# Griffan/VerifyBamID

Measured on AMD Instinct MI355X. Metric: llk_evals_per_sec, higher is better.
Workload: dtype f64; 1 GPU; synthetic pileup 100000 markers x depth 30, --NumPC 4 (BASELINE.json configs[2] shape); parallelism=1 GPU, rccl_world_size=1, launched_by=single process, reads=2999230, active_markers=100000, distinct_codes=42, device=gfx950:sramecc+:xnack-

## Files before the change

### verifybamid_amd/csrc/eval_body.h

```cpp
#ifndef VB2_EVAL_BODY_H_
#define VB2_EVAL_BODY_H_

#include "llk_kernels.h"

#include <hip/hip_runtime.h>

#include "kernel_debug.h"

#include <type_traits>
namespace vb2 {

__device__ __forceinline__ void pair_of(int p, int& g1, int& g2)
{
    g1 = p >> 1;
    const int lo = p & 1;
    g2 = lo + (lo >= g1 ? 1 : 0);
}

__device__ __forceinline__ double wave_sum(double v)
{
    {
        const unsigned hi = (unsigned)__double2hiint(v), lo = (unsigned)__double2loint(v);
        const auto h = __builtin_amdgcn_permlane32_swap(hi, hi, false, false);
        const auto l = __builtin_amdgcn_permlane32_swap(lo, lo, false, false);
// ... 209 lines not shown
__device__ __forceinline__ double prob_entry(double alpha, double p_err, int g1, int g2)
{
    const double p_ok = 1.0 - p_err;
    const double e1 = (double)g1 * (1.0 / 6.0), e2 = (double)g2 * (1.0 / 6.0);
    const double n1 = 1.0 - 0.5 * (double)g1, n2 = 1.0 - 0.5 * (double)g2;
    const double one_minus_alpha = 1.0 - alpha;
    double val = (alpha * e1 + one_minus_alpha * e2) * p_err +
                 (alpha * n1 + one_minus_alpha * n2) * p_ok;
    return val >= 0.0 ? val : __builtin_nan("");
}

__device__ __forceinline__ void initial_gf(double af, double* gf)
{
    af = vmin_f64(vmax_f64(af, 0.00005), 0.99995);
    gf[0] = (1 - af) * (1 - af);
    gf[1] = 2 * (af) * (1 - af);
    gf[2] = af * af;
}


constexpr int kExpTabDoubles = 64 * 32;
constexpr int kPrefetch = 8;
constexpr int kPrefetchL2 = 2;

__device__ __forceinline__ void lane_map(int lane, int& m, int& g)
{
    const int q = (lane >> 2) & 7;
    const int nib = (0x76452310u >> (4 * q)) & 7;
    g = (nib & 1) + 2 * (lane >> 5);
    m = ((nib >> 1) << 2) + (lane & 3);
}
__device__ __forceinline__ int lane_of(int m, int g)
{
    const int idx = ((g & 1) << 2) + (m >> 2);
    const int q = (0x74216530u >> (4 * idx)) & 7;
    return ((g >> 1) << 5) + (q << 2) + (m & 3);
}

__device__ __forceinline__ int lane_xchg_i32(int x, int off, int partner)
{
    if (off == 1) return __builtin_amdgcn_update_dpp(0, x, 0xB1, 0xf, 0xf, true);
    if (off == 2) return __builtin_amdgcn_update_dpp(0, x, 0x4E, 0xf, 0xf, true);
    if (off == 4) {
        const int a = __builtin_amdgcn_update_dpp(0, x, 0x124, 0xf, 0x5, false);
        return __builtin_amdgcn_update_dpp(a, x, 0x12C, 0xf, 0xa, false);
    }
    return __shfl(x, partner, 64);
}
__device__ __forceinline__ double lane_xchg_f64(double x, int off, int partner)
{
    if (off == 1 || off == 2 || off == 4)
        return __hiloint2double(lane_xchg_i32(__double2hiint(x), off, partner), lane_xchg_i32(__double2loint(x), off, partner));
    return __shfl(x, partner, 64);
}

template <int MODE> struct Geom { static constexpr int kMaxWaves = 16, kBlocksPerCU = 1, kWavesPerSimd = 4; };
template <int MODE> struct ModeNp { static constexpr int value = MODE == 2 ? 8 : MODE == 4 ? 1 : MODE == 5 ? 2 : 4; };

struct InlinePoints {
    int count;
    double v[kInlinePointDoubles];
};

struct NoHook {
    __device__ bool on_block() const { return false; }
    __device__ bool mine() const { return false; }
    __device__ void run() {}
    __device__ bool keep_etab() const { return false; }
    __device__ bool prim_in_lds() const { return false; }
    __device__ bool keep_prim() const { return false; }
    __device__ double* sum_stage() const { return nullptr; }
    __device__ uint32_t cache_rec() const { return 0u; }
    __device__ unsigned int* sync_word() const { return nullptr; }
    __device__ bool collect_only() const { return false; }
    __device__ bool no_collect() const { return false; }
};
__host__ __device__ __forceinline__ bool eval_is_dynamic(const DeviceLayout& L, uint32_t nblk, int nwave, int ngrp)
{
    const uint32_t max_tiles_blk = owned_most(L.pd ? 1 : 0, (uint32_t)L.num_mt, nblk);
    return max_tiles_blk * (uint32_t)ngrp <= (uint32_t)(L.dyn_limit * nwave);
}

template <int MODE, bool W16 = false, class Hook = NoHook, bool STREAM = false, int QUEUE = -1, int KSEL = 0,
          bool LCACHE = false, int ESH = 8, bool PD = false, int SPLIT = 0, int RAHEAD = 0>
__device__ __forceinline__ void
eval_body(const DeviceLayout& L, const double* ip_v, const int ip_count, const double* __restrict__ points, int num_valid,
          double* __restrict__ partials, double* __restrict__ llk_out,
          unsigned int* __restrict__ ticket, unsigned long long* __restrict__ done_flag,
          unsigned long long done_seq, const uint32_t blk, const uint32_t nblk,
          unsigned int* __restrict__ batch_done, unsigned int batch_active, const int ngrp_in,
          const unsigned long long tag, const Schedule sch, const bool coherent_points = false,
          const int tid_in = -1, const double* lds_rows = nullptr ,
          Hook hook = Hook())
{
    extern __shared__ __attribute__((aligned(16))) double lds[];
    static_assert(MODE >= 2 && MODE <= 5, "wave shapes 2..5");
    static_assert(!PD || ESH == 8, "probability-domain contexts have no exp table");
    static_assert(!(PD && W16) || ((MODE == 4 || MODE == 5) && STREAM), "8-bit step lists: cohort steps of one and two points");
    static_assert(!SPLIT || (PD && MODE == 2 && QUEUE == 1 && !STREAM && !LCACHE), "split launches: the 8-point shape on the queue");
    constexpr int OSH = PD ? 1 : 0;
    constexpr bool ONEGRP = MODE != 2 || STREAM;
    constexpr int KAF = KSEL > 0 ? 0 : -1;
    constexpr int BTL = MODE == 4 ? 1 : 2;
    constexpr int TPW = MODE == 3 ? 2 : (MODE == 4 || MODE == 5) ? 4 : 1;
    constexpr int SLOTS = 4 / TPW;
    constexpr int NP = SLOTS * BTL;
    constexpr int kReadsAhead = PD ? RAHEAD : 0;
    constexpr bool kOwnSizes = QUEUE == 0 && KSEL == 0 && !PD && !STREAM && (MODE == 3 || MODE == 4) && std::is_same<Hook, NoHook>::value;
    int own_num_code = 0, own_row_bytes = 0, own_num_prim = 0, own_num_mt = 0;
    if constexpr (kOwnSizes) {
        own_num_code = L.num_code; own_row_bytes = L.row_bytes; own_num_prim = L.num_prim; own_num_mt = L.num_mt;
        asm volatile("" : "+s"(own_num_code), "+s"(own_row_bytes), "+s"(own_num_prim), "+s"(own_num_mt));
    }
    const auto l_num_code = [&] { if constexpr (kOwnSizes) return own_num_code; else return L.num_code; };
    const auto l_row_bytes = [&] { if constexpr (kOwnSizes) return own_row_bytes; else return L.row_bytes; };
    const auto l_num_prim = [&] { if constexpr (kOwnSizes) return own_num_prim; else return L.num_prim; };
    const auto l_num_mt = [&] { if constexpr (kOwnSizes) return own_num_mt; else return L.num_mt; };
    const int row_bytes = MODE == 2 ? kRowBytesWide : l_row_bytes();
    const int RS = row_bytes >> 3;
    const int nrow = l_num_code() + 1;
    const int nthread = blockDim.x;
    const int nwave = nthread >> 6;
    const int k = KSEL > 0 ? KSEL : L.num_pc;
    const int stride = 2 * k + 1;
    constexpr int NVS = SPLIT ? SPLIT : 1;
    const int g_per = SPLIT ? (ngrp_in + NVS - 1) / NVS : ngrp_in;
    const int g_lo = SPLIT ? (int)(blk % (uint32_t)NVS) * g_per : 0;
    const int ngrp = ONEGRP ? 1 : SPLIT ? (ngrp_in - g_lo < g_per ? ngrp_in - g_lo : g_per) : ngrp_in;
    const int p_off = g_lo * NP;
    const uint32_t vstep = SPLIT ? nblk / (uint32_t)NVS : 0u, vb0 = SPLIT ? blk / (uint32_t)NVS : blk;
    const double* const known_af_p = KAF == 0 ? nullptr : L.known_af;
    const int NPT = NP * ngrp;
    constexpr int kEtabCopies = (1 << ESH) / 8, kEtabDoubles = PD ? 0 : 64 * kEtabCopies;
    constexpr int kLtabDoubles = PD ? 0 : kLogTabDoubles;
    double* etab = lds;
    double* ltab = lds + kEtabDoubles;
    double* tab = ltab + kLtabDoubles;
    double* red = tab + ngrp * nrow * RS;
    unsigned int* queue = reinterpret_cast<unsigned int*>(red + NVS * NPT);
    double* pts = red + NVS * NPT + 2;
    double* ptq = pts + (size_t)NPT * stride + ((NPT * stride) & 1);
    const size_t prim_off = (size_t)(ptq - lds) + (size_t)NPT * 2 * k;
    double2* prim_lds = reinterpret_cast<double2*>(lds + prim_off + (prim_off & 1));
    double* tile_llk = reinterpret_cast<double*>(prim_lds + l_num_prim());

    const int tid = tid_in >= 0 ? tid_in : (int)threadIdx.x;
    const int lane = tid & 63;
    const int wave = __builtin_amdgcn_readfirstlane(tid >> 6);
    int m, g4;
    lane_map(lane, m, g4);
    const int g = g4 & (SLOTS - 1);
    const int half = TPW == 1 ? 0 : g4 / SLOTS;
    const bool stamp_this = VB2_STAMP_ROUND == 0 || (unsigned)(tag & 0xffffffffull) == (unsigned)VB2_STAMP_ROUND;
#ifdef VB2_ITEM_PROF
    unsigned long long* stamps = nullptr;
#else
    unsigned long long* stamps = (VB2_STAMPS_OF(L) && stamp_this) ? VB2_STAMPS_OF(L) + (size_t)blk * 8 : nullptr;
#endif
    if (stamps && tid == 0) { stamps[0] = wall_clock64(); stamps[4] = 0; }
    if constexpr (SPLIT != 0) {
        if (stamps && tid == 0 && blk != 0u && blk != 20u && blk != 21u) {
            unsigned int xcc;
            asm volatile("s_getreg_b32 %0, hwreg(HW_REG_XCC_ID)" : "=s"(xcc));
            stamps[7] = 1ull + (xcc & 15u);
        }
    }

    const bool collect_only = hook.collect_only();
    if (collect_only && hook.mine()) hook.run();
    if (!collect_only) {
    const bool hook_blk = hook.on_block(), hook_mine = hook.mine();
    unsigned int* const soft_word = PD ? hook.sync_word() : nullptr;
    const bool soft = hook_blk && soft_word != nullptr;
    if (soft && hook_mine) hook.run();
    const int ptid = !soft ? tid : hook_mine ? 0x3fffffff : tid - 64, pnthread = soft ? nthread - 64 : nthread;
    unsigned int soft_gen = 0;
    auto prologue_sync = [&]() {
        if (!soft) { __syncthreads(); return; }
        if (hook_mine) return;
        soft_gen += (unsigned int)(nwave - 1);
        if (lane == 0) __hip_atomic_fetch_add(soft_word, 1u, __ATOMIC_RELAXED, __HIP_MEMORY_SCOPE_WORKGROUP);
        while (__hip_atomic_load(soft_word, __ATOMIC_RELAXED, __HIP_MEMORY_SCOPE_WORKGROUP) < soft_gen) __builtin_amdgcn_s_sleep(1);
        asm volatile("" ::: "memory");
    };
    constexpr bool SPLIT_EARLY = SPLIT != 0 && (kSplitFast & 1) != 0;
    constexpr int kTabSide = 3;
    const int ntab_split = (kAblate & kAblNoTable) ? 0 : (PD ? l_num_prim() - L.num_pair : l_num_prim()) * 6 * NP;
    auto table_inputs = [&](int e, int g0, double2& rec_o, double* al_o) {
        const int pi = e / (6 * NP);
        const int bb = (e - pi * (6 * NP)) / 6;
// ... 264 lines not shown
        for (int i = 0; i < L.stagger; ++i) __builtin_amdgcn_s_sleep(1);
    const bool have_sched = !dyn && sch.off != nullptr;
    uint32_t s_i = 0, s_end = 0;
    if (have_sched) {
        s_i = sch.off[blk * (uint32_t)nwave + (uint32_t)wave];
        s_end = sch.off[blk * (uint32_t)nwave + (uint32_t)wave + 1];
    }
    uint32_t round = 0;
    if (hook_mine && !soft) hook.run();
#ifdef VB2_STAMP_CTRL
    if (stamps && hook_mine && lane == 0) stamps[3] = wall_clock64();
#endif
    typedef __attribute__((address_space(3))) const vuint2 lds_cuint2v;
    constexpr int kPf = (STREAM && !(PD && MODE == 2)) ? kPrefetch : kPrefetchL2;
    RowWord w[kPf];
    constexpr bool PIPE = STREAM && ONEGRP && !LCACHE && QUEUE == 0;
    auto static_item = [&](uint32_t s_pos, uint32_t rnd) -> uint32_t {
        if (have_sched) return s_pos < s_end ? (uint32_t)sch.item[s_pos] : nitem;
        return rnd * (uint32_t)nwave + ((rnd & 1u) ? (uint32_t)(nwave - 1 - wave) : (uint32_t)wave);
    };
    auto tile_of = [&](uint32_t idx_, bool& have_) -> uint32_t {
        const uint32_t it_ = TPW * idx_ + (uint32_t)half;
        have_ = idx_ < nitem && (TPW == 1 || it_ < ntile_blk);
        return have_ ? owned_tile(OSH, blk, nblk, it_) : owned_tile(OSH, blk, nblk, 0u);
    };
    auto draw_item = [&]() -> uint32_t {
        uint32_t nxt = 0;
        if (lane == 0) nxt = atomicAdd(queue, 1u);
        return (uint32_t)__builtin_amdgcn_readfirstlane(nxt);
    };
    auto issue_rows = [&](const vuint2 rec_, bool have_) {
        const uint32_t cb_ = rec_.x * kRowBytes + (uint32_t)m * kLaneBytes;
        const int rows_ = have_ ? (PD ? (int)(((rec_.y >> 16) + (W16 ? 3u : 1u)) >> (W16 ? 2 : 1)) : (int)rec_.y) : 0;
        const int last_ = rows_ > 0 ? rows_ - 1 : 0;
#pragma unroll
        for (int j = 0; j < kPf; ++j) {
            g_cchar* a_ = reinterpret_cast<g_cchar*>(g_codes) + (cb_ + (uint32_t)(j < last_ ? j : last_) * kRowBytes);
            if constexpr (PD) w[j] = *reinterpret_cast<g_cuint*>(a_);
            else w[j] = *reinterpret_cast<g_cuint2*>(a_);
        }
    };
    auto walk_word = [&](const vuint2 w_cur, double* acc, const uint32_t my_tab, const uint32_t my_tab_w16, auto first_tag,
                         const double init) {
        constexpr bool kFirst = decltype(first_tag)::value;
        if constexpr ((kAblate & kAblNoReads) != 0) {
            acc[0] += __hiloint2double((int)((w_cur.x ^ w_cur.y) & 0x000f0000u) | 0x3ff00000, 0);
            return;
        }
#pragma unroll
        for (int j = 0; j < (W16 ? 4 : 2); ++j) {
            double n;
            uint32_t row_addr;
            if constexpr (W16) {
                const uint32_t w2 = (j & 2) ? w_cur.y : w_cur.x;
                const uint32_t idx = (j & 1) ? ((w2 >> 16) & 0xffu) : (w2 & 0xffu);
                const uint32_t hi = __builtin_amdgcn_perm(0x40000000u, w2, (j & 1) ? 0x07030c0cu : 0x07010c0cu);
                n = __hiloint2double((int)hi, 0);
                row_addr = my_tab_w16 + __umul24(idx, (uint32_t)row_bytes);
            } else {
                const uint32_t rw = j ? w_cur.y : w_cur.x;
                n = __hiloint2double((int)(rw & 0xffff0000u), 0);
                row_addr = my_tab + (rw & 0xffffu);
            }
            lds_cdouble2* row = reinterpret_cast<lds_cdouble2*>(row_addr);
#pragma unroll
            for (int i = 0; i < 3 * BTL; ++i) {
                const vdouble2 t = row[i];
                acc[2 * i] = fma(n, t.x, (kFirst && j == 0) ? init : acc[2 * i]);
                acc[2 * i + 1] = fma(n, t.y, (kFirst && j == 0) ? init : acc[2 * i + 1]);
            }
        }
    };
    constexpr bool kEpiAhead = (kReadsAhead == 3 || kReadsAhead == 4) && KSEL > 0 && BTL == 2;
    constexpr int kCqK = !kEpiAhead ? 0 : (kReadsAhead == 3 || KSEL < 2) ? KSEL : 2;
    constexpr int kCq = kEpiAhead ? 2 * kCqK : 1;
    vdouble2 cq[kCq];
    uint32_t cq_addr = 0;
    auto request_cq = [&]() {
#pragma unroll
        for (int i = 0; i < kCq; ++i) cq[i] = *reinterpret_cast<lds_cdouble2*>(cq_addr + (uint32_t)((i & 1) * KSEL + (i >> 1)) * 16u);
    };
    auto walk_pd = [&](const uint32_t w_cur, double* acc, const uint32_t my_tab, auto alt0_tag, auto alt1_tag, auto first_tag, auto pre_tag) {
        constexpr bool kAlt0 = decltype(alt0_tag)::value, kAlt1 = decltype(alt1_tag)::value, kFirst = decltype(first_tag)::value;
        constexpr bool kPre = decltype(pre_tag)::value;
        if constexpr ((kAblate & kAblNoReads) != 0) {
            acc[0] = (kFirst ? 1.0 : acc[0]) * __hiloint2double((int)((w_cur ^ (w_cur >> 16)) & 0x000fu) | 0x3ff00000, 0);
            return;
        }
        if constexpr (kReadsAhead != 0 && !kFirst && (kAblate & kAblNoMul) == 0) {
            vdouble2 t[6 * BTL];
            auto request = [&](const int j) {
                const bool kAlt = j ? kAlt1 : kAlt0;
                const uint32_t row_addr = (kAlt ? my_tab - (uint32_t)kPdAltOffset : my_tab) + (j ? (w_cur >> 16) : (w_cur & 0xffffu));
                lds_cdouble2* row = reinterpret_cast<lds_cdouble2*>(row_addr);
#pragma unroll
                for (int i = 0; i < 3 * BTL; ++i) t[j * 3 * BTL + i] = row[i];
            };
            auto multiply = [&](const int j) {
                const bool kAlt = j ? kAlt1 : kAlt0;
#pragma unroll
                for (int i = 0; i < 3 * BTL; ++i) {
                    const int pt = i / 3, q2 = 2 * (i - 3 * pt);
                    const int a0 = pt * 6 + (kAlt ? 5 - q2 : q2), a1 = pt * 6 + (kAlt ? 4 - q2 : q2 + 1);
                    acc[a0] = acc[a0] * t[j * 3 * BTL + i].x;
                    acc[a1] = acc[a1] * t[j * 3 * BTL + i].y;
                }
            };
            if constexpr (kReadsAhead == 1 || kReadsAhead == 3 || kReadsAhead == 4) {
                request(0); request(1);
                if constexpr (kPre) request_cq();
                multiply(0); multiply(1);
                __builtin_amdgcn_sched_group_barrier(0x100, 6 * BTL + (kPre ? kCq : 0), 0);
                __builtin_amdgcn_sched_group_barrier(0x002, 12 * BTL, 0);
            } else {
#pragma unroll
                for (int j = 0; j < 2; ++j) {
                    request(j);
                    multiply(j);
                    __builtin_amdgcn_sched_group_barrier(0x100, 3 * BTL, 0);
                    __builtin_amdgcn_sched_group_barrier(0x002, 6 * BTL, 0);
                    __builtin_amdgcn_sched_barrier(0);
                }
            }
            return;
        }
#pragma unroll
        for (int j = 0; j < 2; ++j) {
            const bool kAlt = j ? kAlt1 : kAlt0;
            const uint32_t row_addr = (kAlt ? my_tab - (uint32_t)kPdAltOffset : my_tab) + (j ? (w_cur >> 16) : (w_cur & 0xffffu));
            lds_cdouble2* row = reinterpret_cast<lds_cdouble2*>(row_addr);
#pragma unroll
            for (int i = 0; i < 3 * BTL; ++i) {
                const vdouble2 t = row[i];
                const int pt = i / 3, q2 = 2 * (i - 3 * pt);
                const int a0 = pt * 6 + (kAlt ? 5 - q2 : q2), a1 = pt * 6 + (kAlt ? 4 - q2 : q2 + 1);
                if constexpr ((kAblate & kAblNoMul) != 0) {
                    asm volatile("" ::"v"(t.x), "v"(t.y));
                    if (kFirst && j == 0) { acc[a0] = t.x; acc[a1] = t.y; }
                    continue;
                }
                acc[a0] = (kFirst && j == 0) ? t.x : acc[a0] * t.x;
                acc[a1] = (kFirst && j == 0) ? t.y : acc[a1] * t.y;
            }
        }
    };
    auto walk_pd1 = [&](const uint32_t w_cur, double* acc, const uint32_t my_tab, auto first_tag) {
        constexpr bool kFirst = decltype(first_tag)::value;
#pragma unroll
        for (int j = 0; j < 2; ++j) {
            const uint32_t row_addr = my_tab + (j ? (w_cur >> 16) : (w_cur & 0xffffu));
            lds_cdouble2* row = reinterpret_cast<lds_cdouble2*>(row_addr);
#pragma unroll
            for (int i = 0; i < 3 * BTL; ++i) {
                const vdouble2 t = row[i];
                acc[2 * i] = (kFirst && j == 0) ? t.x : acc[2 * i] * t.x;
                acc[2 * i + 1] = (kFirst && j == 0) ? t.y : acc[2 * i + 1] * t.y;
            }
        }
    };
    auto walk_pd8 = [&](const uint32_t w_cur, double* acc, const uint32_t my_tab, auto first_tag, const int step0, const int s1) {
        constexpr bool kFirst = decltype(first_tag)::value;
#pragma unroll
        for (int j = 0; j < 4; ++j) {
            const uint32_t idx = (w_cur >> (8 * j)) & 0xffu;
            const uint32_t base = (step0 + j >= s1) ? my_tab + (uint32_t)kPdAltOffset : my_tab;
            const uint32_t row_addr = base + __umul24(idx, (uint32_t)row_bytes);
            lds_cdouble2* row = reinterpret_cast<lds_cdouble2*>(row_addr);
#pragma unroll
            for (int i = 0; i < 3 * BTL; ++i) {
                const vdouble2 t = row[i];
                acc[2 * i] = (kFirst && j == 0) ? t.x : acc[2 * i] * t.x;
                acc[2 * i + 1] = (kFirst && j == 0) ? t.y : acc[2 * i + 1] * t.y;
            }
        }
    };
    auto marker_lk = [&](const bool live, const uint32_t pos, const double* acc, const double e0, const double e1, const double e2,
// ... 56 lines not shown
                    x01 = exp_nonpos<ESH, true>(a[0], etab_lane); x02 = exp_nonpos<ESH, true>(a[1], etab_lane);
                    x10 = exp_nonpos<ESH, true>(a[2], etab_lane); x12 = exp_nonpos<ESH, true>(a[3], etab_lane);
                    x20 = exp_nonpos<ESH, true>(a[4], etab_lane); x21 = exp_nonpos<ESH, true>(a[5], etab_lane);
                } else {
                    x01 = exp_nonpos<ESH>(a[0], etab_lane); x02 = exp_nonpos<ESH>(a[1], etab_lane);
                    x10 = exp_nonpos<ESH>(a[2], etab_lane); x12 = exp_nonpos<ESH>(a[3], etab_lane);
                    x20 = exp_nonpos<ESH>(a[4], etab_lane); x21 = exp_nonpos<ESH>(a[5], etab_lane);
                }
                double lk;
                if constexpr (PD) {
                    const double o0 = fma(x02, gf2[2], x01 * gf2[1]);
                    const double o1 = fma(x12, gf2[2], x10 * gf2[0]);
                    const double o2 = fma(x21, gf2[1], x20 * gf2[0]);
                    const double off = fma(o2, gf[2], fma(o1, gf[1], o0 * gf[0]));
                    const double dg = fma(e2 * gf2[2], gf[2], fma(e1 * gf2[1], gf[1], (e0 * gf2[0]) * gf[0]));
                    lk = fma(cst_pd, off, dg);
                    if (__builtin_expect(lk < 0x1p-960, 0)) {
                        x01 *= cst_pd; x02 *= cst_pd; x10 *= cst_pd; x12 *= cst_pd; x20 *= cst_pd; x21 *= cst_pd;
                    }
                } else {
                const double s0 = fma(x02, gf2[2], fma(x01, gf2[1], e0 * gf2[0]));
                const double s1 = fma(x12, gf2[2], fma(e1, gf2[1], x10 * gf2[0]));
                const double s2 = fma(e2, gf2[2], fma(x21, gf2[1], x20 * gf2[0]));
                lk = fma(s2, gf[2], fma(s1, gf[1], s0 * gf[0]));
                }
                if (__builtin_expect(lk < 0x1p-960, 0)) {
                    double r = 0;
                    r += e0 * gf[0] * gf2[0];
                    r += x01 * gf[0] * gf2[1];
                    r += x02 * gf[0] * gf2[2];
                    r += x10 * gf[1] * gf2[0];
                    r += e1 * gf[1] * gf2[1];
                    r += x12 * gf[1] * gf2[2];
                    r += x20 * gf[2] * gf2[0];
                    r += x21 * gf[2] * gf2[1];
                    r += e2 * gf[2] * gf2[2];
                    lk = r;
                }
                lk = lk > 0 ? lk : 1.0;
                lk_m[t] = __builtin_amdgcn_frexp_mant(lk);
                lk_e[t] = __builtin_amdgcn_frexp_exp(lk);
            }
        }
    };
    vuint2 rec_nx;
    rec_nx.x = rec_nx.y = 0u;
    double cst_nx = 0.0;
    auto other_const = [&](uint32_t mt_, bool have_) -> double {
        const uint32_t pos_ = mt_ * (uint32_t)kMtMarkers + (uint32_t)m;
        const uint32_t boff_ = ((have_ && pos_ < (uint32_t)L.num_active) ? pos_ : 0u) * 8u;
        return *reinterpret_cast<g_cdouble*>(reinterpret_cast<__attribute__((address_space(1))) const char*>(g_ediag) + boff_);
    };
    const int spare_rank = (wave & 3) ? (wave >> 2) * 3 + (wave & 3) - 1 : (nwave - (nwave >> 2)) + (wave >> 2) - 1;
    int deal_rank = hook_blk ? spare_rank : wave;
    if (VB2_SIMD_DEAL && dyn && nwave == 16 && ONEGRP && nitem <= (uint32_t)(hook_blk ? 15 : 16)) {
        const int n = (int)nitem, sd = wave & 3, sj = wave >> 2;
        int r;
        if (!hook_blk && n <= 8) r = sj == 0 ? sd : sj == 1 ? 7 - sd : n;
        else {
            const int c0 = ((n + 3) >> 2) - (hook_blk ? 1 : 0), nrest = n - c0;
            if (sd == 0) {
                const int j0 = sj - (hook_blk ? 1 : 0);
                r = (j0 >= 0 && j0 < c0) ? nrest + j0 : n;
            } else {
                r = 3 * sj + ((sj & 1) ? 3 - sd : sd - 1);
                if (r >= nrest) r = n;
            }
        }
        deal_rank = r < n ? r : n;
    }
    const uint32_t idx_first = hook_mine ? nitem
                               : have_sched ? (s_i < s_end ? (uint32_t)sch.item[s_i] : nitem)
                                            : (uint32_t)deal_rank;
    if (PIPE && idx_first < nitem) {
        bool h0;
        const uint32_t mt0 = tile_of(idx_first, h0);
        rec_nx = g_rec[mt0];
        cst_nx = other_const(mt0, h0);
        issue_rows(rec_nx, h0);
    }
#ifdef VB2_ITEM_PROF
    unsigned long long ip_sum[8] = {0, 0, 0, 0, 0, 0, 0, 0};
#endif
    for (uint32_t idx = idx_first; idx < nitem;) {
        VB2_IP_T(ip_t0);
        uint32_t grp, unit;
        if (MODE == 2 && QUEUE == 1 && !ONEGRP) {
            unit = ngrp > 1 ? __umulhi(idx, ngrp_magic) : idx;
            grp = idx - unit * (uint32_t)ngrp;
        } else {
            grp = ngrp == 1 ? 0u : (uint32_t)(((float)idx + 0.5f) * inv_nunit);
            if (ngrp != 1) {
                if (grp * nunit > idx) --grp;
                else if ((grp + 1) * nunit <= idx) ++grp;
            }
            unit = idx - grp * nunit;
        }
        const uint32_t vs = SPLIT ? unit % (uint32_t)NVS : 0u;
        const uint32_t it = SPLIT ? unit / (uint32_t)NVS : TPW * unit + (uint32_t)half;
        const bool have_tile = SPLIT ? it < nt_of(vs) : (TPW == 1 || it < ntile_blk);
        const uint32_t mt = owned_tile(OSH, vb0 + vs * vstep, nblk, have_tile ? it : 0u);
        const uint32_t my_tab = tab_addr + (grp * (uint32_t)nrow * (uint32_t)row_bytes + (uint32_t)g * (6 * BTL * 8));
        const uint32_t my_ptq = ptq_addr + (grp * SLOTS + (uint32_t)g) * (uint32_t)(2 * k * BTL * 8);
        const uint32_t my_tab_w16 = (SLOTS == 1 && ONEGRP) ? (uint32_t)((kEtabDoubles + kLogTabDoubles) * sizeof(double)) : my_tab;
        while (!dyn && grp_wave < grp) {
            flush_wave(grp_wave);
            ++grp_wave;
        }
        vuint2 rec;
        if constexpr (LCACHE) rec = *reinterpret_cast<lds_cuint2v*>(hook.cache_rec() + (have_tile ? it : 0u) * 8u);
        else if (PIPE) rec = rec_nx;
        else rec = g_rec[mt];
        VB2_IP_USE(rec.x);
        VB2_IP_T(ip_t1);
        uint32_t idx_next = nitem;
        bool have_next = false;
        uint32_t mt_next = blk;
        vuint2 rec_n2;
        rec_n2.x = rec_n2.y = 0u;
        if (PIPE) {
            idx_next = static_item(s_i + 1, round + 1);
            mt_next = tile_of(idx_next, have_next);
            rec_n2 = g_rec[mt_next];
        }
        const uint32_t pos = mt * (uint32_t)kMtMarkers + (uint32_t)m;
        const bool live = have_tile && pos < (uint32_t)L.num_active;
        const uint32_t boff = (live ? pos : 0u) * 8u;
        auto at = [&](g_cdouble* base_) -> double {
            unsigned long long b_ = (unsigned long long)base_;
            asm volatile("" : "+s"(b_));
            return *reinterpret_cast<g_cdouble*>(reinterpret_cast<__attribute__((address_space(1))) const char*>(b_) + boff);
        };
        const double cst = PIPE ? cst_nx : at(g_ediag);
        const double e0 = at(g_ediag + mp), e1 = at(g_ediag + 2 * mp), e2 = at(g_ediag + 3 * mp);

        double udr[4], mur = 0.0;
#pragma unroll
        for (int kk = 0; kk < 4; ++kk) udr[kk] = (!known_af_p && kk < k) ? at(g_ud + (size_t)kk * mp) : 0.0;
        if (!known_af_p) mur = at(g_mu);

        constexpr bool PEEL = TPW == 1 && !W16 && !PIPE && !LCACHE && QUEUE == 1 && (kAblate & kAblNoReads) == 0;
        double acc[BTL * 6];
        if constexpr (!PEEL && !PD) {
#pragma unroll
            for (int i = 0; i < BTL * 6; ++i) acc[i] = cst;
        }

        if (MODE == 3 && ONEGRP && dyn) {
            if (idx < 4u) __builtin_amdgcn_s_setprio(3);
            else if (idx < 8u) __builtin_amdgcn_s_setprio(2);
            else __builtin_amdgcn_s_setprio(1);
        } else
            __builtin_amdgcn_s_setprio(1);
        const uint32_t cbase = LCACHE ? 0u : rec.x * kRowBytes + (uint32_t)m * kLaneBytes;
        const uint32_t crow = rec.x + (uint32_t)m * kLaneBytes;
        const int steps_ref_v = PD ? (have_tile ? (int)(rec.y & 0xffffu) : 0) : 0;
        const int rows_v = have_tile ? (PD ? (int)(((rec.y >> 16) + (W16 ? 3u : 1u)) >> (W16 ? 2 : 1)) : (int)rec.y) : 0;
        const int steps_ref = (PD && TPW == 1) ? __builtin_amdgcn_readfirstlane(steps_ref_v) : steps_ref_v;
        const int rows = (PD && TPW == 1) ? __builtin_amdgcn_readfirstlane(rows_v) : rows_v;
        const int last_row = rows > 0 ? rows - 1 : 0;
        auto load_row = [&](int j) -> RowWord {
            if constexpr (PD && (kAblate & kAblNoRowLoads) != 0) {
                const uint32_t r0 = ((uint32_t)m * 7u + (uint32_t)j * 2u) % (uint32_t)nrow, r1 = ((uint32_t)m * 7u + (uint32_t)j * 2u + 1u) % (uint32_t)nrow;
                return (r0 * (uint32_t)row_bytes) | ((r1 * (uint32_t)row_bytes) << 16);
            }
            if constexpr (LCACHE && PD) return *reinterpret_cast<lds_cuint*>(crow + (uint32_t)j * kRowBytes);
            else if constexpr (LCACHE) return *reinterpret_cast<lds_cuint2v*>(crow + (uint32_t)j * kRowBytes);
            else {
                g_cchar* a_ = reinterpret_cast<g_cchar*>(g_codes) + (cbase + (uint32_t)(STREAM ? (j < last_row ? j : last_row) : j) * kRowBytes);
                if constexpr (PD) return *reinterpret_cast<g_cuint*>(a_);
                else return *reinterpret_cast<g_cuint2*>(a_);
            }
        };
        if (!PIPE) {
#pragma unroll
            for (int j = 0; j < kPf; ++j) w[j] = load_row(j);
        }
        auto walk_block = [&](const int s0, const bool refill, auto first_tag) {
            constexpr bool kFirstBlock = decltype(first_tag)::value;
#pragma unroll
            for (int u = 0; u < kPf; ++u) {
                if (s0 + u >= rows) break;
                const RowWord w_cur = w[u];
                if (refill) w[u] = load_row(s0 + u + kPf);
                if constexpr (PD) {
                    if constexpr (W16) {
                        if (kFirstBlock && u == 0) walk_pd8(w_cur, acc, my_tab, std::true_type(), (s0 + u) * 4, steps_ref);
                        else walk_pd8(w_cur, acc, my_tab, std::false_type(), (s0 + u) * 4, steps_ref);
                    } else {
                        if (kFirstBlock && u == 0) walk_pd1(w_cur, acc, my_tab, std::true_type());
                        else walk_pd1(w_cur, acc, my_tab, std::false_type());
                    }
                } else {
                    if (kFirstBlock && u == 0) walk_word(w_cur, acc, my_tab, my_tab_w16, std::true_type(), cst);
                    else walk_word(w_cur, acc, my_tab, my_tab_w16, std::false_type(), cst);
                }
            }
        };
        VB2_IP_USE(w[0].x);
        VB2_IP_T(ip_t2);
        if constexpr (PD && TPW > 1 && STREAM) {
            if (__any(rows == 0)) {
                if (rows == 0) {
#pragma unroll
                    for (int i = 0; i < BTL * 6; ++i) acc[i] = 1.0;
                }
            }
            if constexpr (PIPE) {
                const bool more = __any(rows > kPf);
                walk_block(0, more, std::true_type());
                if (more)
                    for (int s0 = kPf; s0 < rows; s0 += kPf) walk_block(s0, true, std::false_type());
                issue_rows(rec_n2, have_next);
                cst_nx = other_const(mt_next, have_next);
                rec_nx = rec_n2;
            } else {
                walk_block(0, true, std::true_type());
                for (int s0 = kPf; s0 < rows; s0 += kPf) walk_block(s0, true, std::false_type());
            }
        } else if constexpr (PD) {
            int r = 0;
            static_assert(kPf == 2, "the ring below has two slots");
            auto row_step_pre = [&](auto slot_tag, auto alt0_tag, auto alt1_tag, auto first_tag, auto pre_tag) {
                constexpr int kSlot = decltype(slot_tag)::value;
                const uint32_t cur = w[kSlot];
                w[kSlot] = load_row(r + kPf);
                walk_pd(cur, acc, my_tab, alt0_tag, alt1_tag, first_tag, pre_tag);
                ++r;
            };
            auto row_step = [&](auto slot_tag, auto alt0_tag, auto alt1_tag, auto first_tag) {
                row_step_pre(slot_tag, alt0_tag, alt1_tag, first_tag, std::false_type());
            };
            const std::integral_constant<int, 0> kS0;
            const std::integral_constant<int, 1> kS1;
            const int rows_ra = steps_ref >> 1;
            const std::false_type kRef;
            const std::true_type kAltT, kFirstT;
            const std::false_type kNotFirst;
            if (rows > 0) {
                if (steps_ref >= 2) row_step(kS0, kRef, kRef, kFirstT);
                else if (steps_ref == 1) row_step(kS0, kRef, kAltT, kFirstT);
                else row_step(kS0, kAltT, kAltT, kFirstT);
            } else {
#pragma unroll
                for (int i = 0; i < BTL * 6; ++i) acc[i] = 1.0;
            }
            auto rows_of_kind = [&](const int end, auto alt_tag) {
                if (r < end && (r & 1)) row_step(kS1, alt_tag, alt_tag, kNotFirst);
                while (r + 1 < end) {
                    row_step(kS0, alt_tag, alt_tag, kNotFirst);
                    row_step(kS1, alt_tag, alt_tag, kNotFirst);
                }
                if (r < end) row_step(kS0, alt_tag, alt_tag, kNotFirst);
            };
            if constexpr (kEpiAhead) {
                cq_addr = my_ptq;
                const int last = rows - 1;
                rows_of_kind(rows_ra < last ? rows_ra : last, kRef);
                if ((steps_ref & 1) && r == rows_ra && r < last) {
                    if (r & 1) row_step(kS1, kRef, kAltT, kNotFirst);
                    else row_step(kS0, kRef, kAltT, kNotFirst);
                }
                rows_of_kind(last, kAltT);
                const std::true_type kPreT;
                if (r < rows) {
                    if (r < rows_ra) {
                        if (r & 1) row_step_pre(kS1, kRef, kRef, kNotFirst, kPreT);
                        else row_step_pre(kS0, kRef, kRef, kNotFirst, kPreT);
                    } else if ((steps_ref & 1) && r == rows_ra) {
                        if (r & 1) row_step_pre(kS1, kRef, kAltT, kNotFirst, kPreT);
                        else row_step_pre(kS0, kRef, kAltT, kNotFirst, kPreT);
                    } else {
                        if (r & 1) row_step_pre(kS1, kAltT, kAltT, kNotFirst, kPreT);
                        else row_step_pre(kS0, kAltT, kAltT, kNotFirst, kPreT);
                    }
                } else
                    request_cq();
            } else {
            rows_of_kind(rows_ra, kRef);
            if ((steps_ref & 1) && r == rows_ra && r < rows) {
                if (r & 1) row_step(kS1, kRef, kAltT, kNotFirst);
                else row_step(kS0, kRef, kAltT, kNotFirst);
            }
            rows_of_kind(rows, kAltT);
            }
            if constexpr (PIPE) {
                issue_rows(rec_n2, have_next);
                cst_nx = other_const(mt_next, have_next);
                rec_nx = rec_n2;
            }
        } else if constexpr (PIPE) {
            const bool more = __any(rows > kPf);
            walk_block(0, more, std::false_type());
            if (more)
                for (int s0 = kPf; s0 < rows; s0 += kPf) walk_block(s0, true, std::false_type());
            issue_rows(rec_n2, have_next);
            cst_nx = other_const(mt_next, have_next);
            rec_nx = rec_n2;
        } else if constexpr (PEEL) {
            if (rows > 0) {
                walk_block(0, true, std::true_type());
                for (int s0 = kPf; s0 < rows; s0 += kPf) walk_block(s0, true, std::false_type());
            } else {
#pragma unroll
                for (int i = 0; i < BTL * 6; ++i) acc[i] = cst;
            }
        } else {
            for (int s0 = 0; s0 < rows; s0 += kPf) walk_block(s0, true, std::false_type());
        }

        __builtin_amdgcn_s_setprio(0);
#ifdef VB2_STAMP_CTRL
        if (stamps && lane == 0 && wave == 1 && !hook_blk) stamps[3] = wall_clock64();
#else
        if (stamps && lane == 0 && wave == 1) stamps[3] = wall_clock64();
#endif
        VB2_IP_USE(acc[0]); VB2_IP_USE(acc[BTL * 6 - 1]);
        VB2_IP_T(ip_t3);
        VB2_IP_USE(e0); VB2_IP_USE(e1); VB2_IP_USE(e2); VB2_IP_USE(mur); VB2_IP_USE(udr[0]); VB2_IP_USE(udr[3]);
        VB2_IP_T(ip_t4);
        double lk_m[BTL];
        int lk_e[BTL];
        marker_lk(live, pos, acc, e0, e1, e2, udr, mur, my_ptq, lk_m, lk_e, cst);
        VB2_IP_USE(lk_m[0]); VB2_IP_USE(lk_m[BTL - 1]);
        VB2_IP_T(ip_t5);
        if (!dyn) {
#pragma unroll
            for (int t = 0; t < BTL; ++t) {
                wave_prod[t].m *= lk_m[t];
                wave_prod[t].e += lk_e[t];
            }
            if (++nfactor == kLazyRenorm) renorm_wave();
            if (have_sched) {
                ++s_i;
                idx = PIPE ? idx_next : (s_i < s_end ? (uint32_t)sch.item[s_i] : nitem);
                continue;
            }
            ++round;
            idx = round * (uint32_t)nwave + ((round & 1u) ? (uint32_t)(nwave - 1 - wave) : (uint32_t)wave);
            continue;
        }
#pragma unroll
        for (int off = 8; off >= 1; off >>= 1) {
            const int partner = lane_of(m ^ off, g4);
#pragma unroll
            for (int t = 0; t < BTL; ++t) {
                lk_m[t] *= lane_xchg_f64(lk_m[t], off, partner);
                lk_e[t] += lane_xchg_i32(lk_e[t], off, partner);
            }
        }
        if (m == 0 && have_tile) {
#pragma unroll
            for (int t = 0; t < BTL; ++t) {
                const size_t o = ((((size_t)grp * NVS + vs) * ntile_blk + it) * NP + g * BTL + t) * 2;
                tile_llk[o] = lk_m[t];
                tile_llk[o + 1] = (double)lk_e[t];
            }
        }
        VB2_IP_T(ip_t6);
        idx = draw_item();
#ifdef VB2_ITEM_PROF
        {
            const unsigned long long ip_t7 = __builtin_readcyclecounter();
            ip_sum[0] += ip_t1 - ip_t0; ip_sum[1] += ip_t2 - ip_t1; ip_sum[2] += ip_t3 - ip_t2; ip_sum[3] += ip_t4 - ip_t3;
            ip_sum[4] += ip_t5 - ip_t4; ip_sum[5] += ip_t6 - ip_t5; ip_sum[6] += ip_t7 - ip_t6; ip_sum[7] += 1;
        }
#endif
    }
#ifdef VB2_ITEM_PROF
    if (VB2_STAMPS_OF(L) && lane == 0 && dyn)
        for (int i = 0; i < 8; ++i) atomicAdd(&VB2_STAMPS_OF(L)[(size_t)blk * 8 + i], ip_sum[i]);
#endif
    if (!dyn) {
        for (uint32_t grp = grp_wave; grp < (uint32_t)ngrp; ++grp) flush_wave(grp);
    }

    if (stamps && lane == 0 && !hook_mine) atomicMax(&stamps[4], wall_clock64());
    const uint32_t nres = dyn ? ntile_blk : (uint32_t)nwave;
    __syncthreads();
    {
        const uint32_t j16 = (uint32_t)lane & 15u;
        for (int b = tid >> 4; b < NVS * NPT; b += nthread >> 4) {
            const int vsb = SPLIT ? b / NPT : 0, bl = b - vsb * NPT;
            const int grp = bl / NP, bb = bl - grp * NP;
            ScaledProd p{1.0, 0.0};
            const uint32_t nres_b = SPLIT ? nt_of((uint32_t)vsb) : nres;
            for (uint32_t i = j16; i < nres_b; i += 16) {
                const size_t o = ((((size_t)grp * NVS + vsb) * nres + i) * NP + bb) * 2;
                p.m *= tile_llk[o];
                p.e += tile_llk[o + 1];
                sp_renorm(p);
            }
            auto row_move = [&](double x, auto ctrl) -> double {
                constexpr int kCtrl = decltype(ctrl)::value;
                return __hiloint2double(__builtin_amdgcn_update_dpp(0, __double2hiint(x), kCtrl, 0xf, 0xf, false),
                                        __builtin_amdgcn_update_dpp(0, __double2loint(x), kCtrl, 0xf, 0xf, false));
            };
            auto row_step = [&](auto ctrl) {
                const double om = row_move(p.m, ctrl), oe = row_move(p.e, ctrl);
                p.m *= om;
                p.e += oe;
            };
            row_step(std::integral_constant<int, 0x140>());
            row_step(std::integral_constant<int, 0x141>());
            row_step(std::integral_constant<int, 0xB1>());
            row_step(std::integral_constant<int, 0x4E>());
            sp_renorm(p);
            if (j16 == 0) red[b] = log_nonneg(p.m) + p.e * 6.93147180559945286227e-01;
        }
    }
    __syncthreads();
    if (VB2_STAMPS_OF(L) && tid == 0) {
        const unsigned long long t5 = wall_clock64();
        if (stamps) stamps[5] = t5;
        if (blk == 0 && nblk > 32 && !hook.no_collect()) VB2_STAMPS_OF(L)[20 * 8 + 7] += t5 - VB2_STAMPS_OF(L)[7];
    }
    }
    auto put_result = [&](int b, double v) {
        if (done_flag) __hip_atomic_store(&llk_out[b], v, __ATOMIC_RELAXED, __HIP_MEMORY_SCOPE_SYSTEM);
        else llk_out[b] = v;
    };
    if (ticket == nullptr) {
        if (tid < NPT) partials[(size_t)tid * nblk + blk] = red[tid];
        return;
    }
    constexpr bool SPLIT_CLASS = SPLIT != 0 && (kSplitFast & 2) != 0;
    unsigned int* const my_ticket = SPLIT_CLASS && ticket ? ticket + blk % (uint32_t)NVS : ticket;
    if constexpr (SPLIT_CLASS) {
        batch_done = ticket ? ticket + NVS : nullptr;
        batch_active = (unsigned int)NVS;
    }
    if (tag == 0) {
        if (tid < NVS * NPT) {
            const int vsb = SPLIT ? tid / NPT : 0, bl = tid - vsb * NPT;
            __hip_atomic_store(&partials[(size_t)(p_off + bl) * nblk + (vb0 + (uint32_t)vsb * vstep)], red[tid],
                               __ATOMIC_RELAXED, __HIP_MEMORY_SCOPE_AGENT);
        }
        unsigned int* last_flag = queue;
        if constexpr (SPLIT_CLASS) {
            if (NVS * NPT <= 64) {
                if (wave == 0) {
                    asm volatile("s_waitcnt vmcnt(0)" ::: "memory");
                    if (lane == 0) {
// ... 146 lines not shown
```

### verifybamid_amd/csrc/kernel_debug.h

```cpp
#ifndef VB2_KERNEL_DEBUG_H_
#define VB2_KERNEL_DEBUG_H_

#ifndef VB2_ABLATE
#define VB2_ABLATE 0
#endif
#ifndef VB2_FLAG_RELEASE
#define VB2_FLAG_RELEASE 1
#endif
#ifndef VB2_SOFT_PROLOGUE
#define VB2_SOFT_PROLOGUE 1
#endif
#ifndef VB2_CTRL_PRIO
#define VB2_CTRL_PRIO 3
#endif
#ifndef VB2_SPLIT_FAST
#define VB2_SPLIT_FAST 3
#endif
#ifndef VB2_READS_AHEAD
#define VB2_READS_AHEAD 0x0111
#endif
#ifndef VB2_SIMD_DEAL
#define VB2_SIMD_DEAL 1
#endif
#ifndef VB2_STAMP_ROUND
#define VB2_STAMP_ROUND 0
#endif

namespace vb2 {
constexpr int kAblNoMap = 1, kAblNoTable = 2, kAblNoItems = 4, kAblNoReads = 8, kAblNoEpi = 16, kAblNoSignal = 32, kAblNoMul = 64, kAblNoRowLoads = 128;
constexpr int kAblate = VB2_ABLATE;
constexpr int kSplitFast = VB2_SPLIT_FAST;
constexpr int kReadsAheadMask = VB2_READS_AHEAD;
constexpr int reads_ahead(int family) { return (kReadsAheadMask >> (4 * family)) & 0xf; }
}

#ifdef VB2_WITH_STAMPS
#define VB2_STAMPS_OF(L) ((L).stamps)
#else
#define VB2_STAMPS_OF(L) (static_cast<unsigned long long*>(nullptr))
#endif

#ifdef VB2_ITEM_PROF
#define VB2_IP_T(var) const unsigned long long var = __builtin_readcyclecounter()
#define VB2_IP_USE(x) asm volatile("" ::"v"(x))
#else
#define VB2_IP_T(var)
#define VB2_IP_USE(x)
#endif

#endif
```

### verifybamid_amd/csrc/llk_kernels.hip

```cpp
#include "llk_kernels.h"

#include <hip/hip_runtime.h>

#include "eval_body.h"
#include "tunables.h"

#include <algorithm>
#include <atomic>
#include <cstring>
#include <type_traits>

namespace vb2 {

template <int MODE, int QUEUE, int KSEL = 0, bool PD = false>
__global__ void __launch_bounds__(Geom<MODE>::kMaxWaves * 64, Geom<MODE>::kWavesPerSimd)
llk_eval_kernel(const DeviceLayout L, const InlinePoints ip, const double* __restrict__ points,
                int num_valid, double* __restrict__ partials, double* __restrict__ llk_out,
                unsigned int* __restrict__ ticket, unsigned long long* __restrict__ done_flag,
                unsigned long long done_seq, int ngrp, unsigned long long tag, const Schedule sch)
{
    eval_body<MODE, false, NoHook, false, QUEUE, KSEL, false, 8, PD, 0, reads_ahead(MODE == 2 ? 1 : 2)>(L, ip.v, ip.count, points, num_valid, partials, llk_out, ticket,
                                                                     done_flag, done_seq, blockIdx.x, gridDim.x, nullptr, 0u, ngrp, tag, sch);
}

template <int KSEL, int S>
__global__ void __launch_bounds__(Geom<2>::kMaxWaves * 64, Geom<2>::kWavesPerSimd)
llk_eval_split_kernel(const DeviceLayout L, const double* __restrict__ points, int num_valid, double* __restrict__ partials,
                      double* __restrict__ llk_out, unsigned int* __restrict__ ticket, unsigned long long* __restrict__ done_flag,
                      unsigned long long done_seq, int ngrp)
{
    eval_body<2, false, NoHook, false, 1, KSEL, false, 8, true, S, reads_ahead(0)>(L, nullptr, 0, points, num_valid, partials, llk_out, ticket, done_flag,
                                                                     done_seq, blockIdx.x, gridDim.x, nullptr, 0u, ngrp, 0ull,
                                                                     Schedule{nullptr, nullptr});
}

#include "resident_kernel.inc"

__global__ void __launch_bounds__(256)
llk_finalize_kernel(const double* __restrict__ partials, int nb, int num_point,
                    double* __restrict__ llk_out, unsigned long long* __restrict__ done_flag,
                    unsigned long long done_seq)
{
    const int lane = threadIdx.x & 63, wave = threadIdx.x >> 6;
    for (int b = wave; b < num_point; b += 4) {
        const double* p = partials + (size_t)b * nb;
        double s = 0;
        for (int base = 0; base < nb; base += 8 * 64) {
            double x[8];
#pragma unroll
            for (int u = 0; u < 8; ++u) {
                const int i = base + u * 64 + lane;
                x[u] = i < nb ? p[i] : 0.0;
            }
#pragma unroll
            for (int u = 0; u < 8; ++u) s += x[u];
        }
        s = wave_sum(s);
        if (lane == 0) {
            if (done_flag) __hip_atomic_store(&llk_out[b], s, __ATOMIC_RELAXED, __HIP_MEMORY_SCOPE_SYSTEM);
            else llk_out[b] = s;
        }
    }
    if (done_flag) {
        asm volatile("s_waitcnt vmcnt(0)" ::: "memory");
        __syncthreads();
        if (threadIdx.x == 0) __hip_atomic_store(done_flag, done_seq, VB2_FLAG_RELEASE ? __ATOMIC_RELEASE : __ATOMIC_RELAXED, __HIP_MEMORY_SCOPE_SYSTEM);
    }
}

bool eval_takes_the_queue(const DeviceLayout& L, int nblk, int nwave, int ngrp)
{
    return eval_is_dynamic(L, (uint32_t)nblk, nwave, ngrp);
}

static size_t split_shmem(const DeviceLayout& L, int grid, int block_waves, int ngrp_total, int ways);

LaunchGeom launch_geom(const DeviceLayout& L, int btl, int ngrp)
{
    const int max_waves = Geom<2>::kMaxWaves;
    const int grid_target = Geom<2>::kBlocksPerCU * L.num_cu;
    (void)btl;
    int bw = (L.num_mt + grid_target - 1) / grid_target;
    bw = bw < 4 ? 4 : (bw > max_waves ? max_waves : bw);
    int grid = (L.num_mt + bw - 1) / bw;
    grid = grid < 1 ? 1 : (grid > grid_target ? grid_target : grid);
    if (L.pd && grid > (L.num_mt >> 1)) grid = L.num_mt >> 1 > 0 ? L.num_mt >> 1 : 1;
    if (L.pd && grid >= 12 && split_shmem(L, grid & ~1, max_waves, kMaxGroups, 2) > (size_t)kLdsLimitBytes)
        grid -= grid % 6;
    if (ngrp > 1) {
        const int items = (int)owned_most(L.pd ? 1 : 0, (uint32_t)L.num_mt, (uint32_t)grid) * ngrp;
        if (items > bw) bw = items > max_waves ? max_waves : items;
    }
    return LaunchGeom{grid, bw};
}

hipError_t raise_lds_limit(const void* fn)
{
    constexpr unsigned kCap = 1024;
    static std::atomic<uintptr_t> keys[kCap];
    int dev = 0;
    hipError_t e = hipGetDevice(&dev);
    if (e != hipSuccess) return e;
    const uintptr_t key = (reinterpret_cast<uintptr_t>(fn) << 8) ^ (uintptr_t)(dev + 1);
    unsigned h = (unsigned)((key * 0x9E3779B97F4A7C15ull) >> 40) % kCap;
    for (unsigned probe = 0; probe < kCap; ++probe, h = (h + 1) % kCap) {
        const uintptr_t seen = keys[h].load(std::memory_order_acquire);
        if (seen == key) return hipSuccess;
        if (seen == 0) break;
    }
    e = hipFuncSetAttribute(fn, hipFuncAttributeMaxDynamicSharedMemorySize, kLdsLimitBytes);
    if (e != hipSuccess) return e;
    for (unsigned probe = 0; probe < kCap; ++probe, h = (h + 1) % kCap) {
        uintptr_t expect = 0;
        if (keys[h].compare_exchange_strong(expect, key, std::memory_order_acq_rel) || expect == key) break;
// ... 336 lines not shown
```

Baseline: 1.080 million evals/s.

## Prefetch next work item's tile record and first code rows during epilogue

Adds an AHEAD template mode for the 8-point probability-domain queue kernel. It draws the next item and loads its tile record before the marker epilogue, then loads its first code-row words afterwards, so global-load latency at the start of each item overlaps the current item's tail. It also precomputes LDS row addresses outside walk_pd, behind an asm barrier, when AHEAD>=2. The cost is extra registers, and the next item is claimed earlier, which can shift how the dynamic queue balances work across blocks.

After: 1.102 million evals/s, median of 6. 2.0% higher.

```diff
diff --git a/verifybamid_amd/csrc/eval_body.h b/verifybamid_amd/csrc/eval_body.h
--- a/verifybamid_amd/csrc/eval_body.h
+++ b/verifybamid_amd/csrc/eval_body.h
@@ -315,7 +315,7 @@
 }
 
 template <int MODE, bool W16 = false, class Hook = NoHook, bool STREAM = false, int QUEUE = -1, int KSEL = 0,
-          bool LCACHE = false, int ESH = 8, bool PD = false, int SPLIT = 0, int RAHEAD = 0>
+          bool LCACHE = false, int ESH = 8, bool PD = false, int SPLIT = 0, int RAHEAD = 0, int AHEAD = 0>
 __device__ __forceinline__ void
 eval_body(const DeviceLayout& L, const double* ip_v, const int ip_count, const double* __restrict__ points, int num_valid,
           double* __restrict__ partials, double* __restrict__ llk_out,
@@ -339,6 +339,9 @@
     constexpr int SLOTS = 4 / TPW;
     constexpr int NP = SLOTS * BTL;
     constexpr int kReadsAhead = PD ? RAHEAD : 0;
+    static_assert(AHEAD == 0 || (PD && MODE == 2 && QUEUE == 1 && !STREAM && !LCACHE && !W16 && std::is_same<Hook, NoHook>::value),
+                  "items requested ahead: the 8-point probability-domain shape on the queue");
+    constexpr bool kAhead = AHEAD != 0 && (kAblate & (kAblNoReads | kAblNoRowLoads)) == 0;
     constexpr bool kOwnSizes = QUEUE == 0 && KSEL == 0 && !PD && !STREAM && (MODE == 3 || MODE == 4) && std::is_same<Hook, NoHook>::value;
     int own_num_code = 0, own_row_bytes = 0, own_num_prim = 0, own_num_mt = 0;
     if constexpr (kOwnSizes) {
@@ -769,7 +772,7 @@
     };
     auto walk_pd = [&](const uint32_t w_cur, double* acc, const uint32_t my_tab, auto alt0_tag, auto alt1_tag, auto first_tag, auto pre_tag) {
         constexpr bool kAlt0 = decltype(alt0_tag)::value, kAlt1 = decltype(alt1_tag)::value, kFirst = decltype(first_tag)::value;
-        constexpr bool kPre = decltype(pre_tag)::value;
+        constexpr bool kPre = ((int)decltype(pre_tag)::value & 1) != 0, kAt = ((int)decltype(pre_tag)::value & 2) != 0;
         if constexpr ((kAblate & kAblNoReads) != 0) {
             acc[0] = (kFirst ? 1.0 : acc[0]) * __hiloint2double((int)((w_cur ^ (w_cur >> 16)) & 0x000fu) | 0x3ff00000, 0);
             return;
@@ -778,7 +781,9 @@
             vdouble2 t[6 * BTL];
             auto request = [&](const int j) {
                 const bool kAlt = j ? kAlt1 : kAlt0;
-                const uint32_t row_addr = (kAlt ? my_tab - (uint32_t)kPdAltOffset : my_tab) + (j ? (w_cur >> 16) : (w_cur & 0xffffu));
+                uint32_t row_addr;
+                if constexpr (kAt) row_addr = j ? my_tab : w_cur;
+                else row_addr = (kAlt ? my_tab - (uint32_t)kPdAltOffset : my_tab) + (j ? (w_cur >> 16) : (w_cur & 0xffffu));
                 lds_cdouble2* row = reinterpret_cast<lds_cdouble2*>(row_addr);
 #pragma unroll
                 for (int i = 0; i < 3 * BTL; ++i) t[j * 3 * BTL + i] = row[i];
@@ -1001,6 +1006,29 @@
 #ifdef VB2_ITEM_PROF
     unsigned long long ip_sum[8] = {0, 0, 0, 0, 0, 0, 0, 0};
 #endif
+    vuint2 rec_ah;
+    rec_ah.x = rec_ah.y = 0u;
+    uint32_t w_ah[3] = {0u, 0u, 0u};
+    auto request_rec_ahead = [&](const uint32_t idx_) {
+        const uint32_t unit_ = ngrp > 1 ? __umulhi(idx_, ngrp_magic) : idx_;
+        const uint32_t vs_ = SPLIT ? unit_ % (uint32_t)NVS : 0u;
+        const uint32_t it_ = SPLIT ? unit_ / (uint32_t)NVS : unit_;
+        const bool have_ = idx_ < nitem && (SPLIT ? it_ < nt_of(vs_) : true);
+        const uint32_t mt_ = have_ ? owned_tile(OSH, vb0 + vs_ * vstep, nblk, it_) : 0u;
+        rec_ah = g_rec[mt_];
+    };
+    auto request_rows_ahead = [&]() {
+        const uint32_t cb_ = rec_ah.x * kRowBytes + (uint32_t)m * kLaneBytes;
+#pragma unroll
+        for (int j = 0; j < 3; ++j)
+            w_ah[j] = *reinterpret_cast<g_cuint*>(reinterpret_cast<g_cchar*>(g_codes) + (cb_ + (uint32_t)j * kRowBytes));
+    };
+    if constexpr (kAhead) {
+        if (idx_first < nitem) {
+            request_rec_ahead(idx_first);
+            request_rows_ahead();
+        }
+    }
     for (uint32_t idx = idx_first; idx < nitem;) {
         VB2_IP_T(ip_t0);
         uint32_t grp, unit;
@@ -1029,6 +1057,7 @@
         vuint2 rec;
         if constexpr (LCACHE) rec = *reinterpret_cast<lds_cuint2v*>(hook.cache_rec() + (have_tile ? it : 0u) * 8u);
         else if (PIPE) rec = rec_nx;
+        else if (kAhead) rec = rec_ah;
         else rec = g_rec[mt];
         VB2_IP_USE(rec.x);
         VB2_IP_T(ip_t1);
@@ -1091,7 +1120,9 @@
                 else return *reinterpret_cast<g_cuint2*>(a_);
             }
         };
-        if (!PIPE) {
+        if constexpr (kAhead) {
+            if constexpr (PD) { w[0] = w_ah[0]; w[1] = w_ah[1]; }
+        } else if (!PIPE) {
 #pragma unroll
             for (int j = 0; j < kPf; ++j) w[j] = load_row(j);
         }
@@ -1143,8 +1174,17 @@
             auto row_step_pre = [&](auto slot_tag, auto alt0_tag, auto alt1_tag, auto first_tag, auto pre_tag) {
                 constexpr int kSlot = decltype(slot_tag)::value;
                 const uint32_t cur = w[kSlot];
-                w[kSlot] = load_row(r + kPf);
-                walk_pd(cur, acc, my_tab, alt0_tag, alt1_tag, first_tag, pre_tag);
+                constexpr bool kAt = kAhead && AHEAD >= 2 && kReadsAhead != 0 && !decltype(first_tag)::value && (kAblate & kAblNoMul) == 0;
+                uint32_t row_a0 = cur, row_a1 = my_tab;
+                if constexpr (kAt) {
+                    row_a0 = (decltype(alt0_tag)::value ? my_tab - (uint32_t)kPdAltOffset : my_tab) + (cur & 0xffffu);
+                    row_a1 = (decltype(alt1_tag)::value ? my_tab - (uint32_t)kPdAltOffset : my_tab) + (cur >> 16);
+                    asm volatile("" : "+v"(row_a0), "+v"(row_a1));
+                }
+                if constexpr (kAhead && decltype(first_tag)::value) w[kSlot] = w_ah[2];
+                else w[kSlot] = load_row(r + kPf);
+                if constexpr (kAt) walk_pd(row_a0, acc, row_a1, alt0_tag, alt1_tag, first_tag, std::integral_constant<int, 2 + (decltype(pre_tag)::value ? 1 : 0)>());
+                else walk_pd(cur, acc, my_tab, alt0_tag, alt1_tag, first_tag, pre_tag);
                 ++r;
             };
             auto row_step = [&](auto slot_tag, auto alt0_tag, auto alt1_tag, auto first_tag) {
@@ -1228,6 +1268,11 @@
             for (int s0 = 0; s0 < rows; s0 += kPf) walk_block(s0, true, std::false_type());
         }
 
+        uint32_t idx_ah = nitem;
+        if constexpr (kAhead) {
+            idx_ah = draw_item();
+            request_rec_ahead(idx_ah);
+        }
         __builtin_amdgcn_s_setprio(0);
 #ifdef VB2_STAMP_CTRL
         if (stamps && lane == 0 && wave == 1 && !hook_blk) stamps[3] = wall_clock64();
@@ -1241,6 +1286,7 @@
         double lk_m[BTL];
         int lk_e[BTL];
         marker_lk(live, pos, acc, e0, e1, e2, udr, mur, my_ptq, lk_m, lk_e, cst);
+        if constexpr (kAhead) request_rows_ahead();
         VB2_IP_USE(lk_m[0]); VB2_IP_USE(lk_m[BTL - 1]);
         VB2_IP_T(ip_t5);
         if (!dyn) {
@@ -1277,7 +1323,8 @@
             }
         }
         VB2_IP_T(ip_t6);
-        idx = draw_item();
+        if constexpr (kAhead) idx = idx_ah;
+        else idx = draw_item();
 #ifdef VB2_ITEM_PROF
         {
             const unsigned long long ip_t7 = __builtin_readcyclecounter();
diff --git a/verifybamid_amd/csrc/kernel_debug.h b/verifybamid_amd/csrc/kernel_debug.h
--- a/verifybamid_amd/csrc/kernel_debug.h
+++ b/verifybamid_amd/csrc/kernel_debug.h
@@ -19,6 +19,9 @@
 #ifndef VB2_READS_AHEAD
 #define VB2_READS_AHEAD 0x0111
 #endif
+#ifndef VB2_ITEM_AHEAD
+#define VB2_ITEM_AHEAD 0x02
+#endif
 #ifndef VB2_SIMD_DEAL
 #define VB2_SIMD_DEAL 1
 #endif
@@ -32,6 +35,8 @@
 constexpr int kSplitFast = VB2_SPLIT_FAST;
 constexpr int kReadsAheadMask = VB2_READS_AHEAD;
 constexpr int reads_ahead(int family) { return (kReadsAheadMask >> (4 * family)) & 0xf; }
+constexpr int kItemAheadMask = VB2_ITEM_AHEAD;
+constexpr int item_ahead(int family) { return (kItemAheadMask >> (4 * family)) & 0xf; }
 }
 
 #ifdef VB2_WITH_STAMPS
diff --git a/verifybamid_amd/csrc/llk_kernels.hip b/verifybamid_amd/csrc/llk_kernels.hip
--- a/verifybamid_amd/csrc/llk_kernels.hip
+++ b/verifybamid_amd/csrc/llk_kernels.hip
@@ -19,7 +19,7 @@
                 unsigned int* __restrict__ ticket, unsigned long long* __restrict__ done_flag,
                 unsigned long long done_seq, int ngrp, unsigned long long tag, const Schedule sch)
 {
-    eval_body<MODE, false, NoHook, false, QUEUE, KSEL, false, 8, PD, 0, reads_ahead(MODE == 2 ? 1 : 2)>(L, ip.v, ip.count, points, num_valid, partials, llk_out, ticket,
+    eval_body<MODE, false, NoHook, false, QUEUE, KSEL, false, 8, PD, 0, reads_ahead(MODE == 2 ? 1 : 2), (MODE == 2 && QUEUE == 1 && PD) ? item_ahead(1) : 0>(L, ip.v, ip.count, points, num_valid, partials, llk_out, ticket,
                                                                      done_flag, done_seq, blockIdx.x, gridDim.x, nullptr, 0u, ngrp, tag, sch);
 }
 
@@ -29,7 +29,7 @@
                       double* __restrict__ llk_out, unsigned int* __restrict__ ticket, unsigned long long* __restrict__ done_flag,
                       unsigned long long done_seq, int ngrp)
 {
-    eval_body<2, false, NoHook, false, 1, KSEL, false, 8, true, S, reads_ahead(0)>(L, nullptr, 0, points, num_valid, partials, llk_out, ticket, done_flag,
+    eval_body<2, false, NoHook, false, 1, KSEL, false, 8, true, S, reads_ahead(0), item_ahead(0)>(L, nullptr, 0, points, num_valid, partials, llk_out, ticket, done_flag,
                                                                      done_seq, blockIdx.x, gridDim.x, nullptr, 0u, ngrp, 0ull,
                                                                      Schedule{nullptr, nullptr});
 }
```
